# allenai/gpv-1

Hardware: AMD Instinct MI355X
Metric: images/sec/node (train step, 480x640, bs32/GPU) (higher is better)
Workload: dtype bf16; 1 GPU; GPV-1 (ResNet-50 + 6+6 DETR layers, 100 queries, RoI head, BERT-base, 3 co-attention, 3 text-decoder layers, V=10000) CocoCaptioning-only train step, dropout 0.1, AdamW; global_batch=32, image=480x640, parallelism=dp1

## Files before the change

gpv-1_amd/csrc/attention.hip:

```cpp
#include "common.h"
#include "../../include/gpv_hip.h"

namespace {

int g_bwd1_mode = tune_env("GPV_ATTN_BWD1", 1);
long g_bwd1_launches = 0;

struct AttnK {
  const void* q; const void* k; const void* v; void* o;
  int64_t q_bs, q_rs, k_bs, k_rs, v_bs, v_rs, o_bs, o_rs;
  int B, H, Sq, Sk, dh, skp, nsplit, sqp;
  float scale;
  const uint8_t* kpm; int causal;
  uint32_t dthresh; float dscale; uint64_t seed; const uint64_t* seed_dev;
  float* lse;
  const void* dout; int64_t do_bs, do_rs;
  void* dq; void* dk; void* dv;
};

constexpr uint32_t ATTN_PAIR_STEP = 0x9E3779B9u;
__device__ __forceinline__ uint32_t attn_row_seed(uint64_t seed, uint64_t row) { return hash_u32(seed, row); }
__device__ __forceinline__ uint32_t attn_pair_bits(uint32_t x) {
  x ^= x >> 16; x = __umul24(x, 0x85EBCBu);
  x ^= x >> 13; x = __umul24(x, 0xC2B2AFu);
  x ^= x >> 16;
  return x;
}
__device__ __forceinline__ int attn_ts(uint32_t dthresh) { return (int)(dthresh >> 16) - 32768; }
__device__ __forceinline__ bool attn_keep_lo(uint32_t w, int ts) { return (int)(short)(w & 0xffffu) >= ts; }
__device__ __forceinline__ bool attn_keep_hi(uint32_t w, int ts) { return ((int)w >> 16) >= ts; }
__device__ __forceinline__ uint32_t attn_drop_bits(uint32_t w, uint32_t ts2) {
  typedef short s16x2 __attribute__((ext_vector_type(2)));
// ... 1006 lines not shown
    T* dvp = reinterpret_cast<T*>(p.dv) + b * p.v_bs + (int64_t)key * p.v_rs + h * p.dh;
#pragma unroll
    for (int dt = 0; dt < DT; ++dt) {
      const int d = dt * 16 + g * 4;
      if (d < p.dh) {
        bf16x4 k4, v4;
#pragma unroll
        for (int i = 0; i < 4; ++i) { k4[i] = (bf16)dkacc[dt][i]; v4[i] = (bf16)dvacc[dt][i]; }
        *reinterpret_cast<bf16x4*>(dkp + d) = k4;
        *reinterpret_cast<bf16x4*>(dvp + d) = v4;
      }
    }
  }
}

template <int DHK, int DHV, int NQT, int NKT, bool CAUSAL>
__global__ __launch_bounds__(QTHR) void attn_bwd1_kernel(AttnK p) {
  using T = bf16;
  if (p.dthresh) p.seed = eff_seed(p.seed, p.seed_dev);
  constexpr int KP = DHK + 8, KC = DHK / 32, DT = DHV / 16, KTW = (NKT + QW - 1) / QW;
  const int sqp = p.sqp, QTP = sqp + 8, skp = p.skp, vtp = skp + 8;
  extern __shared__ __attribute__((aligned(16))) unsigned char smem_raw[];
  bf16* Qh = reinterpret_cast<bf16*>(smem_raw);
  bf16* Dh = Qh + sqp * KP;
  bf16* QTh = Dh + sqp * KP;
  bf16* DTh = QTh + DHV * QTP;
  bf16* KTh = DTh + DHV * QTP;
  bf16* dSb = KTh + DHV * vtp;
  float* lse_s = reinterpret_cast<float*>(dSb + 64 * vtp);
  float* del_s = lse_s + sqp;
  uint32_t* rs_s = reinterpret_cast<uint32_t*>(del_s + sqp);

// ... 14 lines not shown
    const int kt_ = wave + j * QW, key_ = kt_ * 16 + (lane & 15);
    const bool ok = kt_ < nkt && key_ < p.Sk;
#pragma unroll
    for (int kc = 0; kc < KC; ++kc) {
      const int d0 = kc * 32 + g * 8;
      AttnRaw8<T> a, c;
      if (ok && d0 < p.dh) { a.load(kg + (int64_t)key_ * p.k_rs + d0); c.load(vg + (int64_t)key_ * p.v_rs + d0); } else { a.zero(); c.zero(); }
      kh[j][kc] = a.r; vh[j][kc] = c.r;
    }
    kdead[j] = !ok || (p.kpm && p.kpm[(int64_t)b * p.Sk + key_] != 0);
  }

  const T* qg = reinterpret_cast<const T*>(p.q) + b * p.q_bs + h * p.dh;
  const T* dog = reinterpret_cast<const T*>(p.dout) + b * p.do_bs + h * p.dh;
  const T* og = reinterpret_cast<const T*>(p.o) + b * p.o_bs + h * p.dh;
  {
    RowBatch<T, DHK, NQT * 16, QTHR> qr, dr;
    ColBatch<T, DHV, NQT * 16, QTHR> qc, dc;
    qr.load(qg, p.q_rs, p.Sq, sqp, p.dh);
    dr.load(dog, p.do_rs, p.Sq, sqp, p.dh);
    qc.load(qg, p.q_rs, p.Sq, sqp);
    dc.load(dog, p.do_rs, p.Sq, sqp);
    qr.template store<false>(sqp, Qh, nullptr);
    dr.template store<false>(sqp, Dh, nullptr);
    qc.template store<false>(sqp, QTP, QTh, nullptr);
    dc.template store<false>(sqp, QTP, DTh, nullptr);
  }
  {
    ColBatch<T, DHV, NKT * 16, QTHR> kc_;
    kc_.load(kg, p.k_rs, p.Sk, skp);
    kc_.template store<false>(skp, vtp, KTh, nullptr);
  }
  for (int idx = threadIdx.x; idx < 8 * vtp; idx += QTHR)
    reinterpret_cast<bf16x8*>(dSb)[idx] = bf16x8{0, 0, 0, 0, 0, 0, 0, 0};
  for (int r = threadIdx.x; r < sqp; r += QTHR) {
    float dl = 0.f, ls = INFINITY;
    if (r < p.Sq) {
      const T* a = dog + (int64_t)r * p.do_rs;
      const T* c = og + (int64_t)r * p.o_rs;
      for (int d = 0; d < p.dh; d += 8) {
        float u[8], w[8];
        Ld8<T>::ld(a + d, u); Ld8<T>::ld(c + d, w);
#pragma unroll
        for (int e = 0; e < 8; ++e) dl += u[e] * w[e];
      }
      ls = p.lse[((int64_t)b * p.H + h) * p.Sq + r];
    }
    lse_s[r] = -ls * 1.4426950408889634f; del_s[r] = dl;
    rs_s[r] = p.dthresh ? attn_row_seed(p.seed, ((uint64_t)b * p.H + h) * p.Sq + r) : 0u;
  }
  __syncthreads();

  const float c2k = p.scale * 1.4426950408889634f;
// ... 195 lines not shown
  if (nsplit > (nkt + QW - 1) / QW) nsplit = (nkt + QW - 1) / QW;
  if (nsplit < 1) nsplit = 1;
  p.nsplit = nsplit;
  hipLaunchKernelGGL(fn, dim3(nsplit * bh), dim3(QTHR), lds, st, p);
  GPV_CHECK_LAUNCH();
  return 0;
}
template <int DHK, int DHV>
int launch_kv2(AttnK p, hipStream_t st) {
  if (p.Sq > 320) return -1;
  p.sqp = ((p.Sq + 31) / 32) * 32;
  if (p.sqp <= 128) return p.causal ? launch_kv2_c<DHK, DHV, 8, true>(p, st) : launch_kv2_c<DHK, DHV, 8, false>(p, st);
  return p.causal ? launch_kv2_c<DHK, DHV, 20, true>(p, st) : launch_kv2_c<DHK, DHV, 20, false>(p, st);
}

template <int DHK, int DHV, int NQT, int NKT, bool CAUSAL>
int launch_bwd1_c(AttnK p, hipStream_t st) {
  constexpr int KP = DHK + 8;
  const int QTP = p.sqp + 8, vtp = p.skp + 8;
  const size_t lds = ((size_t)2 * p.sqp * KP + (size_t)2 * DHV * QTP + (size_t)DHV * vtp + (size_t)64 * vtp) * 2 + (size_t)3 * p.sqp * sizeof(float);
  if (lds > 160 * 1024) return -1;
  auto fn = attn_bwd1_kernel<DHK, DHV, NQT, NKT, CAUSAL>;
  static size_t attr = 0;
  if (lds > 64 * 1024 && lds > attr) {
    hipError_t e = hipFuncSetAttribute(reinterpret_cast<const void*>(fn), hipFuncAttributeMaxDynamicSharedMemorySize, (int)lds);
    if (e != hipSuccess) { (void)hipGetLastError(); return (int)e; }
    attr = lds;
  }
  p.nsplit = 1;
  hipLaunchKernelGGL(fn, dim3(p.B * p.H), dim3(QTHR), lds, st, p);
  GPV_CHECK_LAUNCH();
  ++g_bwd1_launches;
  return 0;
}
template <int DHK, int DHV>
int launch_bwd1(AttnK p, hipStream_t st) {
  if (p.Sq > 320 || p.skp > 320) return -1;
  p.sqp = ((p.Sq + 31) / 32) * 32;
  const bool q8 = p.sqp <= 128, k8 = p.skp <= 128;
  if (p.causal) return (q8 && k8) ? launch_bwd1_c<DHK, DHV, 8, 8, true>(p, st) : -1;
  if (q8 && k8) return launch_bwd1_c<DHK, DHV, 8, 8, false>(p, st);
  if constexpr (DHK == 32) {
    if (q8) return launch_bwd1_c<DHK, DHV, 8, 20, false>(p, st);
    if (!k8) return launch_bwd1_c<DHK, DHV, 20, 20, false>(p, st);
  }
  return -1;
}
int dispatch_bwd1(const AttnK& p, hipStream_t st) {
  if (g_bwd1_mode == 0 || (g_bwd1_mode == 1 && p.B * p.H < 128)) return -1;
  switch (p.dh) {
    case 32: return launch_bwd1<32, 32>(p, st);
    case 48: return launch_bwd1<64, 48>(p, st);
    case 64: return launch_bwd1<64, 64>(p, st);
    case 96: return launch_bwd1<96, 96>(p, st);
// ... 609 lines not shown
  return elems * 2 * (sizeof(T) == 4 ? 2 : 1) + (size_t)p.skp * sizeof(float) <= 160 * 1024;
}

int fill(const gpv_attn_args* a, AttnK& p) {
  if (!a || !a->q || !a->k || !a->v || a->Sk <= 0 || a->Sq <= 0) return (int)hipErrorInvalidValue;
  p.q = a->q; p.k = a->k; p.v = a->v; p.o = a->o;
  p.q_bs = a->q_bs; p.q_rs = a->q_rs; p.k_bs = a->k_bs; p.k_rs = a->k_rs; p.v_bs = a->v_bs; p.v_rs = a->v_rs;
  p.o_bs = a->o_bs; p.o_rs = a->o_rs;
  p.B = a->B; p.H = a->H; p.Sq = a->Sq; p.Sk = a->Sk; p.dh = a->dh;
  p.skp = ((a->Sk + 63) / 64) * 64;
  p.scale = a->scale; p.kpm = a->kpm; p.causal = a->causal;
  p.dthresh = a->drop_p > 0.f ? drop_thresh(a->drop_p) : 0u;
  p.dscale = a->drop_p > 0.f ? 1.f / (1.f - a->drop_p) : 1.f;
  p.seed = a->seed; p.seed_dev = gpvk::g_seed_dev; p.lse = a->lse;
  p.dout = a->dout; p.do_bs = a->do_bs; p.do_rs = a->do_rs; p.dq = a->dq; p.dk = a->dk; p.dv = a->dv;
  return 0;
}
}

namespace gpvk {
int attn_bwd1_mode(int set) { const int prev = g_bwd1_mode; g_bwd1_mode = set; return prev; }
long attn_bwd1_launches(long set) { const long prev = g_bwd1_launches; if (set >= 0) g_bwd1_launches = set; return prev; }
}

extern "C" int gpv_attention_fwd(const gpv_attn_args* a, void* stream) {
  AttnK p{};
  int e = fill(a, p);
  if (e) return e;
  if (!a->o) return (int)hipErrorInvalidValue;
  hipStream_t st = reinterpret_cast<hipStream_t>(stream);
// ... 29 lines not shown
  if ((reinterpret_cast<uintptr_t>(a->q) | reinterpret_cast<uintptr_t>(a->k) | reinterpret_cast<uintptr_t>(a->o)) & 7) return (int)hipErrorInvalidValue;
  if (!a->v || (reinterpret_cast<uintptr_t>(a->v) & 1) || (reinterpret_cast<uintptr_t>(bias) & 3) || a->v_rs < a->H * a->dh || a->q_rs < a->H * a->dh ||
      a->k_rs < a->H * a->dh) return (int)hipErrorInvalidValue;
  QkvK xk{reinterpret_cast<const bf16*>(xp), reinterpret_cast<const bf16*>(x), x_bs, x_rs, reinterpret_cast<const bf16*>(w), bias};
  hipStream_t st = reinterpret_cast<hipStream_t>(stream);
  if (p.skp <= 128) return p.skp == 128 ? launch_qkv<8, true>(p, xk, st) : launch_qkv<8, false>(p, xk, st);
  return p.skp == 320 ? launch_qkv<20, true>(p, xk, st) : launch_qkv<20, false>(p, xk, st);
}

extern "C" int gpv_attention_bwd(const gpv_attn_args* a, void* stream) {
  AttnK p{};
  int e = fill(a, p);
  if (e) return e;
  if (!a->o || !a->dout || !a->dq || !a->dk || !a->dv || !a->lse) return (int)hipErrorInvalidValue;
  hipStream_t st = reinterpret_cast<hipStream_t>(stream);
  const bool f32 = a->dtype == GPV_F32;
  if (!(f32 ? q_short_fits<float, 1>(p) : q_short_fits<bf16, 1>(p))) {
    e = f32 ? dispatch_long<float, 1>(p, st) : dispatch_long<bf16, 1>(p, st);
    if (e) return e;
    return f32 ? dispatch_kvl<float>(p, st) : dispatch_kvl<bf16>(p, st);
  }
  if (a->dtype != GPV_F32) {
    e = dispatch_bwd1(p, st);
    if (e >= 0) return e;
  }
  e = a->dtype == GPV_F32 ? dispatch_q<float, 1>(p, st) : dispatch_q<bf16, 1>(p, st);
  if (e) return e;
  return a->dtype == GPV_F32 ? dispatch_kv<float>(p, st) : dispatch_kv<bf16>(p, st);
}
```

gpv-1_amd/hip.py:

```python
import ctypes as C
import os
import threading

import torch

BF16, F32 = 0, 1
ACT_NONE, ACT_RELU, ACT_GELU = 0, 1, 2
KMAJOR, TRANS = 0, 1

_LIB = None
TUNING = os.environ.get('GPV_TUNING_LIB', '0') == '1'
_LIB_PATH = os.environ.get('GPV_HIP_LIB') or os.path.join(os.path.dirname(os.path.abspath(__file__)), 'csrc',
                                                          'libgpv_hip_tuning.so' if TUNING else 'libgpv_hip.so')


class GemmArgs(C.Structure):
    _fields_ = [('A', C.c_void_p), ('B', C.c_void_p), ('C', C.c_void_p),
                ('M', C.c_int), ('N', C.c_int), ('K', C.c_int), ('batch', C.c_int),
                ('lda', C.c_int64), ('ldb', C.c_int64), ('ldc', C.c_int64),
                ('sA', C.c_int64), ('sB', C.c_int64), ('sC', C.c_int64),
                ('layoutA', C.c_int), ('layoutB', C.c_int), ('dtype_in', C.c_int), ('dtype_out', C.c_int),
                ('alpha', C.c_float), ('rowscale', C.c_void_p), ('bias', C.c_void_p),
                ('res', C.c_void_p), ('ldr', C.c_int64), ('sR', C.c_int64),
                ('relu_mask', C.c_void_p), ('ldm', C.c_int64),
# ... 9 lines not shown
                ('KH', C.c_int), ('KW', C.c_int), ('SH', C.c_int), ('SW', C.c_int), ('PH', C.c_int), ('PW', C.c_int),
                ('dtype_in', C.c_int), ('dtype_out', C.c_int),
                ('rowscale', C.c_void_p), ('bias', C.c_void_p), ('res', C.c_void_p), ('relu_mask', C.c_void_p),
                ('act', C.c_int), ('split_k', C.c_int), ('workspace', C.c_void_p), ('workspace_bytes', C.c_int64),
                ('y_mask_bits', C.c_void_p), ('relu_mask_bits', C.c_void_p)]


class AttnArgs(C.Structure):
    _fields_ = [('q', C.c_void_p), ('k', C.c_void_p), ('v', C.c_void_p), ('o', C.c_void_p),
                ('q_bs', C.c_int64), ('q_rs', C.c_int64), ('k_bs', C.c_int64), ('k_rs', C.c_int64),
                ('v_bs', C.c_int64), ('v_rs', C.c_int64), ('o_bs', C.c_int64), ('o_rs', C.c_int64),
                ('B', C.c_int), ('H', C.c_int), ('Sq', C.c_int), ('Sk', C.c_int), ('dh', C.c_int),
                ('scale', C.c_float), ('kpm', C.c_void_p), ('causal', C.c_int),
                ('drop_p', C.c_float), ('seed', C.c_uint64), ('lse', C.c_void_p), ('dtype', C.c_int),
                ('dout', C.c_void_p), ('do_bs', C.c_int64), ('do_rs', C.c_int64),
                ('dq', C.c_void_p), ('dk', C.c_void_p), ('dv', C.c_void_p)]


class TTProblem(C.Structure):
    _fields_ = [('A', C.c_void_p), ('B', C.c_void_p), ('C', C.c_void_p), ('a_rowsum', C.c_void_p),
                ('M', C.c_int), ('N', C.c_int), ('K', C.c_int), ('lda', C.c_int), ('ldb', C.c_int), ('ldc', C.c_int)]


class FoldProblem(C.Structure):
    _fields_ = [('partials', C.c_void_p), ('out0', C.c_void_p), ('out1', C.c_void_p), ('nblk', C.c_int), ('cols', C.c_int)]


class ConvWgradProblem(C.Structure):
    _fields_ = [('x', C.c_void_p), ('dy', C.c_void_p), ('dw', C.c_void_p), ('rowscale', C.c_void_p)] + \
               [(k, C.c_int) for k in ('B', 'IH', 'IW', 'Cs', 'Cin', 'OH', 'OW', 'Cout', 'KH', 'KW', 'SH', 'SW', 'PH', 'PW')]

# ... 305 lines not shown
        raise ValueError('attention_qkv_fwd: xp and x must share one row layout (the library takes ONE pair of strides for both)')
    a = _attn_args(q, k, v, o, strides, B, H, S, S, 32, scale, kpm, False, drop_p, seed, lse)
    _chk(lib().gpv_attention_qkv_fwd(C.byref(a), _p(xp), _p(x), C.c_int64(S * x.stride(0)), C.c_int64(x.stride(0)), _p(w), _p(_f32(bias)),
                                     _stream()), 'gpv_attention_qkv_fwd')


def attention_bwd(q, k, v, o, dout, dq, dk, dv, strides, do_strides, B, H, Sq, Sk, dh, scale, kpm=None,
                  causal=False, drop_p=0.0, seed=0, lse=None):
    a = _attn_args(q, k, v, o, strides, B, H, Sq, Sk, dh, scale, kpm, causal, drop_p, seed, lse)
    a.dout = _p(dout)
    a.do_bs, a.do_rs = do_strides
    a.dq, a.dk, a.dv = _p(dq), _p(dk), _p(dv)
    _chk(lib().gpv_attention_bwd(C.byref(a), _stream()), 'gpv_attention_bwd')


def linear_layernorm_fwd(a, w, bias, x, gamma, beta, s, y, mean, rstd, rows, eps, drop_p=0.0, seed=0, pos=None, y2=None):
    if (pos is None) != (y2 is None):
        raise ValueError('pos and y2 come together')
    if any(t.dtype != torch.bfloat16 for t in (a, w, x, s, y)):
        raise TypeError('linear_layernorm_fwd: bf16 activations and weight')
    _chk(lib().gpv_linear_layernorm_fwd(_p(a), _p(w), _p(_f32(bias)), _p(x), _p(_f32(gamma)), _p(_f32(beta)), _p(s), _p(y), _p(_f32(mean)),
                                        _p(_f32(rstd)), C.c_int(rows), C.c_int(w.shape[1]), C.c_int(w.shape[0]), C.c_float(eps), C.c_float(drop_p), C.c_uint64(seed),
                                        _p(pos), C.c_int(0 if pos is None else pos.numel() // w.shape[0]), _p(y2), _stream()), 'gpv_linear_layernorm_fwd')


def layernorm_fwd(x, s, gamma, beta, y, mean, rstd, rows, cols, eps, drop_p=0.0, seed=0, pos=None, y2=None):
    if (pos is None) != (y2 is None):
        raise ValueError('layernorm_fwd: pos and y2 come together')
    if pos is not None and (pos.dtype != x.dtype or y2.dtype != x.dtype or pos.numel() % cols != 0):
        raise TypeError('layernorm_fwd: pos / y2 in the activation dtype, whole rows')
# ... 314 lines not shown
```

gpv-1_amd/ops.py:

```python
import math

import os
import weakref

import torch
from torch.autograd import Function

from . import hip

ACT_NONE, ACT_RELU, ACT_GELU = hip.ACT_NONE, hip.ACT_RELU, hip.ACT_GELU


class Runtime:
    def __init__(self):
        self.dtype = torch.bfloat16
        self.weights_epoch = 0
        self.static_epoch = 0
        self.seed = 0x5EED
        self.seed_explicit = False
        self._ctr = 0
        self.cache = {}
        self.backward_milestone = None
        self.split = None
        self.seed_dev = None
# ... 786 lines not shown
            elif dsr is not None and ds is None:
                dxr = dxr.clone()
            dxr = ch.done(dxr)
        return ((dxr if ctx.needs_input_grad[0] else None), (dsr if ctx.needs_input_grad[1] else None)) + (None,) * (nin - 2)


PROJ_LN = os.environ.get('GPV_PROJ_LN', '1') != '0'
PROJ_LN_MIN_ROWS = int(os.environ.get('GPV_PROJ_LN_MIN_ROWS', '2048'))


def proj_layernorm_ok(w, x):
    return (PROJ_LN and RT.dtype == torch.bfloat16 and w.K == 256 and w.N == 256 and x.shape[-1] == 256 and w.bias is not None
            and x.numel() // 256 >= PROJ_LN_MIN_ROWS)


class ProjAddLayerNormFn(Function):

    @staticmethod
    def forward(ctx, x, a, w, gamma, beta, eps, drop_p, chain=None, pos=None, pos_param=None):
        ctx.chain = chain.join() if (chain is not None and ctx.needs_input_grad[0]) else None
        ctx.set_materialize_grads(False)
        cols = x.shape[-1]
        x2 = _c(_as_compute(x)).reshape(-1, cols)
        a2 = _c(_as_compute(a)).reshape(-1, w.K)
        rows = x2.shape[0]
        s2 = torch.empty_like(x2)
        y = torch.empty_like(x2)
        mean = torch.empty(rows, device=x.device, dtype=torch.float32)
        rstd = torch.empty_like(mean)
        seed = RT.next_seed() if drop_p > 0 else 0
# ... 11 lines not shown
    @staticmethod
    def backward(ctx, dy, dy2=None):
        nin = 10
        if dy is None and dy2 is None:
            return (None,) * nin
        x2, s2, mean, rstd, a2 = ctx.saved_tensors
        rows, cols = x2.shape
        if dy2 is not None:
            _pos_sink(ctx.pos_param, _c(_as_compute(dy2)).reshape(rows, cols), rows, cols)
        d1, d2 = _two_grads(dy, dy2, rows, cols)
        dx = torch.empty_like(x2)
        ds = torch.empty_like(x2) if ctx.drop_p > 0 else None
        _ln_backward(d1, d2, x2, s2, ctx.gamma, ctx.beta, mean, rstd, dx, ds, rows, cols, ctx.drop_p, ctx.seed)
        dxr = dx.reshape(ctx.shape)
        if ctx.chain is not None and ctx.needs_input_grad[0]:
            ch = ctx.chain
            if ch.acc is not None:
                t = torch.empty_like(dx)
                hip.add(dx, _c(ch.acc).reshape(rows, cols), t, t.numel())
                dxr = t.reshape(ctx.shape)
            elif ds is None:
                dxr = dxr.clone()
            dxr = ch.done(dxr)
        da = _linear_backward(ctx.w, a2, ds if ds is not None else dx, None, ctx.needs_input_grad[1], ctx.ashape)
        return ((dxr if ctx.needs_input_grad[0] else None), da) + (None,) * (nin - 2)


def proj_add_layernorm(x, a, w, gamma, beta, eps, drop_p=0.0, chain=None, pos=None, pos_param=None):
    return ProjAddLayerNormFn.apply(x, a, w, gamma, beta, eps, drop_p, chain, pos, pos_param)


FFN_FUSED = os.environ.get('GPV_FFN_FUSED', '0') == '1'


class FFNBlockFn(Function):

    @staticmethod
    def forward(ctx, x, w1, w2, gamma, beta, eps, drop_p, pos=None, pos_param=None):
# ... 157 lines not shown

    @staticmethod
    def backward(ctx, do):
        w, B, H, S, kpm, drop_p = ctx.meta[:6]
        E = w.K
        xp2, x2, qk, v, o, lse = ctx.saved_tensors
        do = _c(_as_compute(do))
        dqk, dv = torch.empty_like(qk), torch.empty_like(v)
        hip.attention_bwd(qk[:, :E], qk[:, E:], v, o, do, dqk[:, :E], dqk[:, E:], dv, ctx.st, (S * E, E), B, H, S, S, E // H, ctx.scale,
                          kpm=kpm, drop_p=drop_p, seed=ctx.seed, lse=lse)
        dx = _linear_backward(W(w.weight, w.bias, 2 * E, 3 * E), x2, dv, ctx.cv, ctx.needs_input_grad[2], ctx.x_shape)
        dxp = _linear_backward(W(w.weight, w.bias, 0, 2 * E), xp2, dqk, ctx.cq, ctx.needs_input_grad[1], ctx.xp_shape)
        return None, dxp, dx, None


def attention_qkv(xp, x, w, B, H, S, kpm=None, drop_p=0.0, chains=(None, None)):
    dummy = None
    if torch.is_grad_enabled() and not (xp.requires_grad or x.requires_grad) and (w.weight.requires_grad or (w.bias is not None and w.bias.requires_grad)):
        dummy = _dummy(x.device)
    return SelfAttnQKVFn.apply((w, B, H, S, kpm, drop_p, chains[0], chains[1]), xp, x, dummy)


class AddFn(Function):

    @staticmethod
    def forward(ctx, a, b):
        ctx.set_materialize_grads(False)
        a2, b2 = _c(_as_compute(a)), _c(_as_compute(b))
        y = torch.empty_like(a2)
        cols = a2.shape[-1]
# ... 169 lines not shown
```

gpv-1_amd/transformer.py:

```python
import os

import torch
import torch.nn as nn

from . import ops
from .ops import W

HOIST_KV = os.environ.get('GPV_HOIST_KV', '1') != '0'


class LinearP(nn.Module):

    def __init__(self, in_features, out_features, bias=True):
        super().__init__()
        ref = nn.Linear(in_features, out_features, bias=bias)
        self.weight = nn.Parameter(ref.weight.detach().clone())
        self.bias = nn.Parameter(ref.bias.detach().clone()) if bias else None
        self.in_features, self.out_features = in_features, out_features

    def forward(self, x, act=ops.ACT_NONE, drop_p=0.0, out_f32=False, chain=None):
        return ops.linear(x, W(self.weight, self.bias), act, drop_p, out_f32, chain)


def ffn_block(x, l1, l2, norm, drop_p, pos=None, pos_param=None):
# ... 19 lines not shown

class MultiheadAttention(nn.Module):

    def __init__(self, embed_dim, num_heads, dropout=0.0):
        super().__init__()
        self.embed_dim, self.num_heads, self.dropout = embed_dim, num_heads, dropout
        self.head_dim = embed_dim // num_heads
        self.in_proj_weight = nn.Parameter(torch.empty(3 * embed_dim, embed_dim))
        self.in_proj_bias = nn.Parameter(torch.zeros(3 * embed_dim))
        self.out_proj = LinearP(embed_dim, embed_dim)
        nn.init.xavier_uniform_(self.in_proj_weight)
        nn.init.constant_(self.out_proj.bias, 0.)

    def forward(self, q_in, k_in, v_in, B, Sq, Sk, key_padding_mask=None, causal=False, chains=(None, None, None), kv=None, out_drop=0.0,
                no_proj=False):
        E = self.embed_dim
        w, b = self.in_proj_weight, self.in_proj_bias
        cq, ck, cv = chains
        if kv is not None:
            k_all, kcol, v_all, vcol, sk, sv = kv
            q = ops.linear(q_in, W(w, b, 0, E), chain=cq)
            if k_all is v_all:
                bufs, roles, sinks = [q, k_all], ((0, 0), (1, kcol), (1, vcol)), (None, sk)
            else:
                bufs, roles, sinks = [q, k_all, v_all], ((0, 0), (1, kcol), (2, vcol)), (None, sk, sv)
            o = ops.attention(bufs, roles, B, self.num_heads, Sq, Sk, self.head_dim, kpm=key_padding_mask,
                              causal=causal, drop_p=self.dropout if self.training else 0.0,
                              sinks=sinks if (sk is not None or sv is not None) else None)
            return o if no_proj else self.out_proj(o, drop_p=out_drop)
        if q_in is k_in and k_in is v_in:
            bufs = [ops.linear(q_in, W(w, b, 0, 3 * E), chain=cq)]
            roles = ((0, 0), (0, E), (0, 2 * E))
        elif q_in is k_in:
            if Sq == Sk and ops.attention_qkv_ok(E, self.num_heads, Sq, causal, B):
                o = ops.attention_qkv(q_in, v_in, W(w, b, 0, 3 * E), B, self.num_heads, Sq, kpm=key_padding_mask,
                                      drop_p=self.dropout if self.training else 0.0, chains=(cq, cv))
                return o if no_proj else self.out_proj(o, drop_p=out_drop)
            bufs = [ops.linear(q_in, W(w, b, 0, 2 * E), chain=cq), ops.linear(v_in, W(w, b, 2 * E, 3 * E), chain=cv)]
            roles = ((0, 0), (0, E), (1, 0))
        elif k_in is v_in:
            bufs = [ops.linear(q_in, W(w, b, 0, E), chain=cq), ops.linear(k_in, W(w, b, E, 3 * E), chain=ck)]
            roles = ((0, 0), (1, 0), (1, E))
        else:
            bufs = [ops.linear(q_in, W(w, b, 0, E), chain=cq), ops.linear(k_in, W(w, b, E, 2 * E), chain=ck),
                    ops.linear(v_in, W(w, b, 2 * E, 3 * E), chain=cv)]
            roles = ((0, 0), (1, 0), (2, 0))
        o = ops.attention(bufs, roles, B, self.num_heads, Sq, Sk, self.head_dim, kpm=key_padding_mask, causal=causal,
                          drop_p=self.dropout if self.training else 0.0)
        return o if no_proj else self.out_proj(o, drop_p=out_drop)


class TransformerEncoderLayer(nn.Module):
    def __init__(self, d_model, nhead, dim_feedforward=2048, dropout=0.1):
        super().__init__()
        self.self_attn = MultiheadAttention(d_model, nhead, dropout=dropout)
        self.linear1 = LinearP(d_model, dim_feedforward)
        self.linear2 = LinearP(dim_feedforward, d_model)
        self.norm1 = LayerNormP(d_model)
        self.norm2 = LayerNormP(d_model)
        self.p = dropout

    def forward(self, src, qk, pos, B, S, kpm):
        p = self.p if self.training else 0.0
        ch = ops.grad_chain(src)
        o = self.self_attn(qk, qk, src, B, S, S, kpm, chains=(ch, ch, ch), no_proj=True)
        src = self.norm1.proj(src, o, self.self_attn.out_proj, p, chain=ch)
        return ffn_block(src, self.linear1, self.linear2, self.norm2, p, pos=pos)

    def forward_pre(self, src, pos, B, S, kpm, pos_grad=False):
        p = self.p if self.training else 0.0
        if pos_grad:
            s2 = self.norm1(src)
            qk = ops.add(s2, pos)
        else:
            s2, qk = self.norm1(src, pos=pos)
        src = ops.add(src, self.self_attn(qk, qk, s2, B, S, S, kpm, out_drop=p))
        s2 = self.norm2(src)
        return ops.add(src, self.linear2(self.linear1(s2, ops.ACT_RELU, p), drop_p=p))


class TransformerDecoderLayer(nn.Module):
    def __init__(self, d_model, nhead, dim_feedforward=2048, dropout=0.1):
        super().__init__()
        self.self_attn = MultiheadAttention(d_model, nhead, dropout=dropout)
        self.multihead_attn = MultiheadAttention(d_model, nhead, dropout=dropout)
        self.linear1 = LinearP(d_model, dim_feedforward)
        self.linear2 = LinearP(dim_feedforward, d_model)
        self.norm1 = LayerNormP(d_model)
        self.norm2 = LayerNormP(d_model)
        self.norm3 = LayerNormP(d_model)
        self.p = dropout

    def forward(self, tgt, tgt_qp, memory, mem_pos, qpos, qpos_param, B, Q, S, kpm, mem_chain=None, emit=True, kv=None):
        p = self.p if self.training else 0.0
        ch = ops.grad_chain(tgt)
        o = self.self_attn(tgt_qp, tgt_qp, tgt, B, Q, Q, chains=(None, None, ch), no_proj=True)
        tgt, tq = self.norm1.proj(tgt, o, self.self_attn.out_proj, p, chain=ch, pos=qpos, pos_param=qpos_param)
        a = self.multihead_attn(tq, mem_pos, memory, B, Q, S, kpm, chains=(None, mem_chain, mem_chain), kv=kv, no_proj=True)
        tgt = self.norm2.proj(tgt, a, self.multihead_attn.out_proj, p)
        if not emit:
            return ffn_block(tgt, self.linear1, self.linear2, self.norm3, p), None
        return ffn_block(tgt, self.linear1, self.linear2, self.norm3, p, pos=qpos, pos_param=qpos_param)

    def forward_pre(self, tgt, memory, mem_pos, qpos, qpos_param, B, Q, S, kpm):
        p = self.p if self.training else 0.0
        t2, tq = self.norm1(tgt, pos=qpos, pos_param=qpos_param)
        tgt = ops.add(tgt, self.self_attn(tq, tq, t2, B, Q, Q, out_drop=p))
        t2, tq = self.norm2(tgt, pos=qpos, pos_param=qpos_param)
        tgt = ops.add(tgt, self.multihead_attn(tq, mem_pos, memory, B, Q, S, kpm, out_drop=p))
        t2 = self.norm3(tgt)
        return ops.add(tgt, self.linear2(self.linear1(t2, ops.ACT_RELU, p), drop_p=p))


class TransformerEncoder(nn.Module):
# ... 124 lines not shown
```

include/gpv_hip.h:

```cpp
#ifndef GPV_HIP_H
#define GPV_HIP_H
#include <stdint.h>
#ifdef __cplusplus
extern "C" {
#endif

#define GPV_BF16 0
#define GPV_F32 1

#define GPV_ACT_NONE 0
#define GPV_ACT_RELU 1
#define GPV_ACT_GELU 2

#define GPV_KMAJOR 0
#define GPV_TRANS 1

int gpv_abi_version(void);
int gpv_build_id(char* buf, int cap);

#define GPV_TT_GROUP_MAX 48
typedef struct {
  const void* A; const void* B; float* C; float* a_rowsum;
  int M, N, K;
  int lda, ldb, ldc;
// ... 122 lines not shown
#endif
int gpv_stem_pool(const void* x, const void* w, const float* shift, void* y, int B, int Hp, int Wp, int CH, int CW, int PH, int PW,
                  void* stream);

typedef struct {
  const void* q; const void* k; const void* v; void* o;
  int64_t q_bs, q_rs, k_bs, k_rs, v_bs, v_rs, o_bs, o_rs;
  int B, H, Sq, Sk, dh;
  float scale;
  const uint8_t* kpm; int causal;
  float drop_p; uint64_t seed;
  float* lse;
  int dtype;
  const void* dout; int64_t do_bs, do_rs;
  void* dq; void* dk; void* dv;
} gpv_attn_args;
int gpv_attention_fwd(const gpv_attn_args* a, void* stream);
int gpv_attention_bwd(const gpv_attn_args* a, void* stream);
int gpv_attention_qkv_fwd(const gpv_attn_args* a, const void* xp, const void* x, int64_t x_bs, int64_t x_rs, const void* w,
                          const float* bias, void* stream);

int gpv_layernorm_fwd(const void* x, const void* s, const float* gamma, const float* beta, void* y,
                      float* mean, float* rstd, int rows, int cols, float eps, float drop_p,
                      uint64_t seed, int dtype, void* stream);
int gpv_layernorm_bwd(const void* dy, const void* x, const void* s, const float* gamma,
                      const float* mean, const float* rstd, void* dx, void* ds, float* dgamma,
                      float* dbeta, int rows, int cols, float drop_p, uint64_t seed, int dtype,
                      void* stream);
int gpv_layernorm_pos_fwd(const void* x, const void* s, const float* gamma, const float* beta, void* y, float* mean, float* rstd,
                          int rows, int cols, float eps, float drop_p, uint64_t seed, const void* pos, int pos_rows, void* y2,
                          int dtype, void* stream);
// ... 71 lines not shown
```

Baseline: 2142 images/sec.

## Fuse out-projection input-gradient GEMM into attention backward prologue

Adds a PROJ variant of the attention backward kernel that computes dO = dZ·Wo^T per head inside the prologue with MFMA, so the separate dx GEMM and the dO round trip through global memory go away. A new autograd function, AttnSublayerFn, wraps attention, the out-projection and the residual LayerNorm as one sublayer for the encoder and decoder layers. Each block now rereads the full 256-wide dZ row and a slice of the weight, which adds redundant loads across heads. The PROJ path only applies to bf16 attention with 8 heads of 32, non-causal, and sequence lengths up to 320; other cases fall back to the old path.

```diff
diff --git a/gpv-1_amd/csrc/attention.hip b/gpv-1_amd/csrc/attention.hip
--- a/gpv-1_amd/csrc/attention.hip
+++ b/gpv-1_amd/csrc/attention.hip
@@ -16,6 +16,7 @@
   float* lse;
   const void* dout; int64_t do_bs, do_rs;
   void* dq; void* dk; void* dv;
+  const void* wt;
 };
 
 constexpr uint32_t ATTN_PAIR_STEP = 0x9E3779B9u;
@@ -1052,8 +1053,9 @@
   }
 }
 
-template <int DHK, int DHV, int NQT, int NKT, bool CAUSAL>
+template <int DHK, int DHV, int NQT, int NKT, bool CAUSAL, bool PROJ = false>
 __global__ __launch_bounds__(QTHR) void attn_bwd1_kernel(AttnK p) {
+  static_assert(!PROJ || (DHK == 32 && DHV == 32 && !CAUSAL), "the projection prologue is built for 8 heads of 32");
   using T = bf16;
   if (p.dthresh) p.seed = eff_seed(p.seed, p.seed_dev);
   constexpr int KP = DHK + 8, KC = DHK / 32, DT = DHV / 16, KTW = (NKT + QW - 1) / QW;
@@ -1098,7 +1100,54 @@
   const T* qg = reinterpret_cast<const T*>(p.q) + b * p.q_bs + h * p.dh;
   const T* dog = reinterpret_cast<const T*>(p.dout) + b * p.do_bs + h * p.dh;
   const T* og = reinterpret_cast<const T*>(p.o) + b * p.o_bs + h * p.dh;
-  {
+  if constexpr (PROJ) {
+    constexpr int KD = 256, KCX = KD / 32, NR = (NQT + QW - 1) / QW;
+    const int li = lane & 15, nqt = sqp >> 4;
+    RowBatch<T, DHK, NQT * 16, QTHR> qr;
+    ColBatch<T, DHV, NQT * 16, QTHR> qc;
+    qr.load(qg, p.q_rs, p.Sq, sqp, p.dh);
+    qc.load(qg, p.q_rs, p.Sq, sqp);
+    const T* wg = reinterpret_cast<const T*>(p.wt) + (int64_t)(h * 32 + li) * KD + g * 8;
+    const T* zg = reinterpret_cast<const T*>(p.dout) + b * p.do_bs + g * 8;
+    bf16x8 wf[2][KCX], nz[KCX];
+#pragma unroll
+    for (int dt = 0; dt < 2; ++dt)
+#pragma unroll
+      for (int kc = 0; kc < KCX; ++kc) wf[dt][kc] = *reinterpret_cast<const bf16x8*>(wg + dt * 16 * KD + kc * 32);
+    auto fetch = [&](int t) {
+      const T* zr = zg + (int64_t)min(t * 16 + li, p.Sq - 1) * p.do_rs;
+#pragma unroll
+      for (int kc = 0; kc < KCX; ++kc) nz[kc] = *reinterpret_cast<const bf16x8*>(zr + kc * 32);
+    };
+    fetch(wave);
+    qr.template store<false>(sqp, Qh, nullptr);
+    qc.template store<false>(sqp, QTP, QTh, nullptr);
+#pragma unroll
+    for (int r = 0; r < NR; ++r) {
+      const int t = wave + r * QW;
+      if (t < nqt) {
+        bf16x8 zf[KCX];
+#pragma unroll
+        for (int kc = 0; kc < KCX; ++kc) zf[kc] = nz[kc];
+        if (r + 1 < NR) fetch(t + QW);
+        f32x4 acc[2] = {f32x4{0.f, 0.f, 0.f, 0.f}, f32x4{0.f, 0.f, 0.f, 0.f}};
+#pragma unroll
+        for (int kc = 0; kc < KCX; ++kc)
+#pragma unroll
+          for (int dt = 0; dt < 2; ++dt) acc[dt] = mfma16(wf[dt][kc], zf[kc], acc[dt]);
+        const int q = t * 16 + li;
+#pragma unroll
+        for (int dt = 0; dt < 2; ++dt) {
+          bf16x4 d4;
+#pragma unroll
+          for (int i = 0; i < 4; ++i) d4[i] = q < p.Sq ? (bf16)acc[dt][i] : (bf16)0.f;
+          *reinterpret_cast<bf16x4*>(Dh + q * KP + dt * 16 + g * 4) = d4;
+#pragma unroll
+          for (int i = 0; i < 4; ++i) DTh[(dt * 16 + g * 4 + i) * QTP + q] = d4[i];
+        }
+      }
+    }
+  } else {
     RowBatch<T, DHK, NQT * 16, QTHR> qr, dr;
     ColBatch<T, DHV, NQT * 16, QTHR> qc, dc;
     qr.load(qg, p.q_rs, p.Sq, sqp, p.dh);
@@ -1117,10 +1166,11 @@
   }
   for (int idx = threadIdx.x; idx < 8 * vtp; idx += QTHR)
     reinterpret_cast<bf16x8*>(dSb)[idx] = bf16x8{0, 0, 0, 0, 0, 0, 0, 0};
+  if constexpr (PROJ) __syncthreads();
   for (int r = threadIdx.x; r < sqp; r += QTHR) {
     float dl = 0.f, ls = INFINITY;
     if (r < p.Sq) {
-      const T* a = dog + (int64_t)r * p.do_rs;
+      const T* a = PROJ ? Dh + r * KP : dog + (int64_t)r * p.do_rs;
       const T* c = og + (int64_t)r * p.o_rs;
       for (int d = 0; d < p.dh; d += 8) {
         float u[8], w[8];
@@ -1346,13 +1396,13 @@
   return p.causal ? launch_kv2_c<DHK, DHV, 20, true>(p, st) : launch_kv2_c<DHK, DHV, 20, false>(p, st);
 }
 
-template <int DHK, int DHV, int NQT, int NKT, bool CAUSAL>
+template <int DHK, int DHV, int NQT, int NKT, bool CAUSAL, bool PROJ = false>
 int launch_bwd1_c(AttnK p, hipStream_t st) {
   constexpr int KP = DHK + 8;
   const int QTP = p.sqp + 8, vtp = p.skp + 8;
   const size_t lds = ((size_t)2 * p.sqp * KP + (size_t)2 * DHV * QTP + (size_t)DHV * vtp + (size_t)64 * vtp) * 2 + (size_t)3 * p.sqp * sizeof(float);
   if (lds > 160 * 1024) return -1;
-  auto fn = attn_bwd1_kernel<DHK, DHV, NQT, NKT, CAUSAL>;
+  auto fn = attn_bwd1_kernel<DHK, DHV, NQT, NKT, CAUSAL, PROJ>;
   static size_t attr = 0;
   if (lds > 64 * 1024 && lds > attr) {
     hipError_t e = hipFuncSetAttribute(reinterpret_cast<const void*>(fn), hipFuncAttributeMaxDynamicSharedMemorySize, (int)lds);
@@ -1370,6 +1420,15 @@
   if (p.Sq > 320 || p.skp > 320) return -1;
   p.sqp = ((p.Sq + 31) / 32) * 32;
   const bool q8 = p.sqp <= 128, k8 = p.skp <= 128;
+  if (p.wt) {
+    if constexpr (DHK == 32) {
+      if (p.causal) return -1;
+      if (q8 && k8) return launch_bwd1_c<DHK, DHV, 8, 8, false, true>(p, st);
+      if (q8) return launch_bwd1_c<DHK, DHV, 8, 20, false, true>(p, st);
+      if (!k8) return launch_bwd1_c<DHK, DHV, 20, 20, false, true>(p, st);
+    }
+    return -1;
+  }
   if (p.causal) return (q8 && k8) ? launch_bwd1_c<DHK, DHV, 8, 8, true>(p, st) : -1;
   if (q8 && k8) return launch_bwd1_c<DHK, DHV, 8, 8, false>(p, st);
   if constexpr (DHK == 32) {
@@ -2009,6 +2068,7 @@
   p.dscale = a->drop_p > 0.f ? 1.f / (1.f - a->drop_p) : 1.f;
   p.seed = a->seed; p.seed_dev = gpvk::g_seed_dev; p.lse = a->lse;
   p.dout = a->dout; p.do_bs = a->do_bs; p.do_rs = a->do_rs; p.dq = a->dq; p.dk = a->dk; p.dv = a->dv;
+  p.wt = nullptr;
   return 0;
 }
 }
@@ -2068,6 +2128,15 @@
   if (e) return e;
   if (!a->o || !a->dout || !a->dq || !a->dk || !a->dv || !a->lse) return (int)hipErrorInvalidValue;
   hipStream_t st = reinterpret_cast<hipStream_t>(stream);
+  if (a->proj_wt) {
+    if (a->dtype != GPV_BF16 || a->dh != 32 || a->H * a->dh != 256 || a->Sq > 320 || a->Sk > 320 || a->causal || a->proj_ld != 256)
+      return GPV_NOT_TAKEN;
+    if ((a->do_rs & 7) || (a->do_bs & 7) || a->do_rs < 256 || a->do_bs < (int64_t)a->Sq * a->do_rs) return (int)hipErrorInvalidValue;
+    if ((reinterpret_cast<uintptr_t>(a->dout) | reinterpret_cast<uintptr_t>(a->proj_wt)) & 15) return (int)hipErrorInvalidValue;
+    p.wt = a->proj_wt;
+    e = dispatch_bwd1(p, st);
+    return e >= 0 ? e : GPV_NOT_TAKEN;
+  }
   const bool f32 = a->dtype == GPV_F32;
   if (!(f32 ? q_short_fits<float, 1>(p) : q_short_fits<bf16, 1>(p))) {
     e = f32 ? dispatch_long<float, 1>(p, st) : dispatch_long<bf16, 1>(p, st);
diff --git a/gpv-1_amd/hip.py b/gpv-1_amd/hip.py
--- a/gpv-1_amd/hip.py
+++ b/gpv-1_amd/hip.py
@@ -47,7 +47,8 @@
                 ('scale', C.c_float), ('kpm', C.c_void_p), ('causal', C.c_int),
                 ('drop_p', C.c_float), ('seed', C.c_uint64), ('lse', C.c_void_p), ('dtype', C.c_int),
                 ('dout', C.c_void_p), ('do_bs', C.c_int64), ('do_rs', C.c_int64),
-                ('dq', C.c_void_p), ('dk', C.c_void_p), ('dv', C.c_void_p)]
+                ('dq', C.c_void_p), ('dk', C.c_void_p), ('dv', C.c_void_p),
+                ('proj_wt', C.c_void_p), ('proj_ld', C.c_int64)]
 
 
 class TTProblem(C.Structure):
@@ -383,6 +384,27 @@
     _chk(lib().gpv_attention_bwd(C.byref(a), _stream()), 'gpv_attention_bwd')
 
 
+NOT_TAKEN = -1
+
+
+def attention_bwd_proj(q, k, v, o, dz, wt, dq, dk, dv, strides, B, H, Sq, Sk, dh, scale, kpm=None, causal=False, drop_p=0.0, seed=0,
+                       lse=None):
+    if dz.dim() != 2 or wt.dim() != 2 or dz.stride(1) != 1 or wt.stride(1) != 1 or dz.dtype != q.dtype or wt.dtype != q.dtype:
+        return False
+    if dz.shape[0] != B * Sq or dz.shape[1] != H * dh or tuple(wt.shape) != (H * dh, H * dh):
+        return False
+    a = _attn_args(q, k, v, o, strides, B, H, Sq, Sk, dh, scale, kpm, causal, drop_p, seed, lse)
+    a.dout = _p(dz)
+    a.do_bs, a.do_rs = Sq * dz.stride(0), dz.stride(0)
+    a.dq, a.dk, a.dv = _p(dq), _p(dk), _p(dv)
+    a.proj_wt, a.proj_ld = _p(wt), wt.stride(0)
+    err = lib().gpv_attention_bwd(C.byref(a), _stream())
+    if err == NOT_TAKEN:
+        return False
+    _chk(err, 'gpv_attention_bwd (proj)')
+    return True
+
+
 def linear_layernorm_fwd(a, w, bias, x, gamma, beta, s, y, mean, rstd, rows, eps, drop_p=0.0, seed=0, pos=None, y2=None):
     if (pos is None) != (y2 is None):
         raise ValueError('pos and y2 come together')
diff --git a/gpv-1_amd/ops.py b/gpv-1_amd/ops.py
--- a/gpv-1_amd/ops.py
+++ b/gpv-1_amd/ops.py
@@ -824,6 +824,17 @@
             and x.numel() // 256 >= PROJ_LN_MIN_ROWS)
 
 
+def _residual_grad(ch, dx, dx_is_dz, shape):
+    dxr = dx.reshape(shape)
+    if ch.acc is not None:
+        t = torch.empty_like(dx)
+        hip.add(dx, _c(ch.acc).reshape(dx.shape), t, t.numel())
+        dxr = t.reshape(shape)
+    elif dx_is_dz:
+        dxr = dxr.clone()
+    return ch.done(dxr)
+
+
 class ProjAddLayerNormFn(Function):
 
     @staticmethod
@@ -865,14 +876,7 @@
         _ln_backward(d1, d2, x2, s2, ctx.gamma, ctx.beta, mean, rstd, dx, ds, rows, cols, ctx.drop_p, ctx.seed)
         dxr = dx.reshape(ctx.shape)
         if ctx.chain is not None and ctx.needs_input_grad[0]:
-            ch = ctx.chain
-            if ch.acc is not None:
-                t = torch.empty_like(dx)
-                hip.add(dx, _c(ch.acc).reshape(rows, cols), t, t.numel())
-                dxr = t.reshape(ctx.shape)
-            elif ds is None:
-                dxr = dxr.clone()
-            dxr = ch.done(dxr)
+            dxr = _residual_grad(ctx.chain, dx, ds is None, ctx.shape)
         da = _linear_backward(ctx.w, a2, ds if ds is not None else dx, None, ctx.needs_input_grad[1], ctx.ashape)
         return ((dxr if ctx.needs_input_grad[0] else None), da) + (None,) * (nin - 2)
 
@@ -1060,6 +1064,120 @@
         return None, dxp, dx, None
 
 
+ATTN_PROJ_BWD = os.environ.get('GPV_ATTN_PROJ_BWD', '1') != '0'
+
+
+def attention_proj_ok(E, H, Sq, Sk, causal, B):
+    return (ATTN_PROJ_BWD and RT.dtype == torch.bfloat16 and E == 256 and H == 8 and 0 < Sq <= 320 and 0 < Sk <= 320 and not causal
+            and B * H >= 64)
+
+
+class AttnSublayerFn(Function):
+
+    @staticmethod
+    def forward(ctx, meta, x, dummy, *ins):
+        front, w, gamma, beta, eps, drop_p, chain, pos, pos_param = meta
+        E = w.K
+        if front[0] == 'qkv':
+            _, wi, B, H, Sq, kpm, adrop, chain_qk, chain_v = front
+            Sk, dh = Sq, E // H
+            xp2 = _c(_as_compute(ins[0])).reshape(-1, E)
+            xv2 = _c(_as_compute(ins[1])).reshape(-1, E)
+            M = xp2.shape[0]
+            qk = torch.empty(M, 2 * E, device=xp2.device, dtype=RT.dtype)
+            v = torch.empty(M, E, device=xp2.device, dtype=RT.dtype)
+            bufs, roles = (qk, v), ((0, 0), (0, E), (1, 0))
+            ctx.cq = chain_qk.join() if (chain_qk is not None and ctx.needs_input_grad[3]) else None
+            ctx.cv = chain_v.join() if (chain_v is not None and ctx.needs_input_grad[4]) else None
+            ctx.in_shapes = (ins[0].shape, ins[1].shape)
+            extra = (xp2, xv2)
+        else:
+            _, roles, B, H, Sq, Sk, dh, kpm, adrop, sinks = front
+            bufs = tuple(_c(_as_compute(b)) for b in ins)
+            extra = ()
+        (qi, qo), (ki, ko), (vi, vo) = roles
+        qb, kb, vb = bufs[qi], bufs[ki], bufs[vi]
+        o = torch.empty(B * Sq, E, device=qb.device, dtype=RT.dtype)
+        lse = torch.empty(B, H, Sq, device=qb.device, dtype=torch.float32)
+        st = ((Sq * qb.shape[1], qb.shape[1]), (Sk * kb.shape[1], kb.shape[1]), (Sk * vb.shape[1], vb.shape[1]), (Sq * E, E))
+        aseed = RT.next_seed() if adrop > 0 else 0
+        scale = 1.0 / math.sqrt(dh)
+        if front[0] == 'qkv':
+            hip.attention_qkv_fwd(xp2, xv2, wi.lp(), wi.bias_f32(), qk[:, :E], qk[:, E:], v, o, st, B, H, Sq, scale, kpm=kpm, drop_p=adrop,
+                                  seed=aseed, lse=lse)
+        else:
+            hip.attention_fwd(qb[:, qo:], kb[:, ko:], vb[:, vo:], o, st, B, H, Sq, Sk, dh, scale, kpm=kpm, drop_p=adrop, seed=aseed, lse=lse)
+        ctx.chain = chain.join() if (chain is not None and ctx.needs_input_grad[1]) else None
+        ctx.set_materialize_grads(False)
+        x2 = _c(_as_compute(x)).reshape(-1, E)
+        rows = x2.shape[0]
+        s2 = torch.empty_like(x2)
+        y = torch.empty_like(x2)
+        mean = torch.empty(rows, device=x.device, dtype=torch.float32)
+        rstd = torch.empty_like(mean)
+        seed = RT.next_seed() if drop_p > 0 else 0
+        p2 = None if pos is None else _pos_rows(pos, E)
+        y2 = None if pos is None else torch.empty_like(x2)
+        hip.linear_layernorm_fwd(o, w.lp(), w.bias_f32(), x2, None if gamma is None else gamma.detach(), None if beta is None else beta.detach(),
+                                 s2, y, mean, rstd, rows, eps, drop_p, seed, pos=p2, y2=y2)
+        ctx.meta, ctx.aseed, ctx.seed, ctx.st, ctx.scale, ctx.shape, ctx.nbuf = meta, aseed, seed, st, scale, x.shape, len(bufs)
+        ctx.geom = (roles, B, H, Sq, Sk, dh, kpm, adrop)
+        ctx.save_for_backward(x2, s2, mean, rstd, o, lse, *bufs, *extra)
+        if pos is None:
+            return y.reshape(x.shape)
+        return y.reshape(x.shape), y2.reshape(x.shape)
+
+    @staticmethod
+    def backward(ctx, dy, dy2=None):
+        front, w, gamma, beta, eps, drop_p, _, _, pos_param = ctx.meta
+        nin = 3 + (2 if front[0] == 'qkv' else ctx.nbuf)
+        if dy is None and dy2 is None:
+            return (None,) * nin
+        x2, s2, mean, rstd, o, lse, *rest = ctx.saved_tensors
+        bufs, extra = rest[:ctx.nbuf], rest[ctx.nbuf:]
+        roles, B, H, Sq, Sk, dh, kpm, adrop = ctx.geom
+        rows, cols = x2.shape
+        if dy2 is not None:
+            _pos_sink(pos_param, _c(_as_compute(dy2)).reshape(rows, cols), rows, cols)
+        d1, d2 = _two_grads(dy, dy2, rows, cols)
+        dx = torch.empty_like(x2)
+        ds = torch.empty_like(x2) if drop_p > 0 else None
+        _ln_backward(d1, d2, x2, s2, gamma, beta, mean, rstd, dx, ds, rows, cols, drop_p, ctx.seed)
+        dxr = dx.reshape(ctx.shape)
+        if ctx.chain is not None and ctx.needs_input_grad[1]:
+            dxr = _residual_grad(ctx.chain, dx, ds is None, ctx.shape)
+        dz = ds if ds is not None else dx
+        _linear_backward(w, o, dz, None, False, None)
+        (qi, qo), (ki, ko), (vi, vo) = roles
+        sinks = front[9] if (front[0] == 'bufs' and front[9] is not None) else (None,) * len(bufs)
+        grads = [torch.empty_like(b) if s is None else s.slot(b) for b, s in zip(bufs, sinks)]
+        q, k, v = bufs[qi][:, qo:], bufs[ki][:, ko:], bufs[vi][:, vo:]
+        dq, dk, dv = grads[qi][:, qo:], grads[ki][:, ko:], grads[vi][:, vo:]
+        akw = dict(kpm=kpm, drop_p=adrop, seed=ctx.aseed, lse=lse)
+        if not (w.mirror_ok() and hip.attention_bwd_proj(q, k, v, o, dz, w.lpT(), dq, dk, dv, ctx.st, B, H, Sq, Sk, dh, ctx.scale, **akw)):
+            do = torch.empty_like(o)
+            w.dx_gemm(dz, do, rows)
+            hip.attention_bwd(q, k, v, o, do, dq, dk, dv, ctx.st, (Sq * cols, cols), B, H, Sq, Sk, dh, ctx.scale, **akw)
+        gx = dxr if ctx.needs_input_grad[1] else None
+        if front[0] == 'qkv':
+            wi, E = front[1], cols
+            xp2, xv2 = extra
+            dxv = _linear_backward(W(wi.weight, wi.bias, 2 * E, 3 * E), xv2, grads[1], ctx.cv, ctx.needs_input_grad[4], ctx.in_shapes[1])
+            dxp = _linear_backward(W(wi.weight, wi.bias, 0, 2 * E), xp2, grads[0], ctx.cq, ctx.needs_input_grad[3], ctx.in_shapes[0])
+            return None, gx, None, dxp, dxv
+        for s_ in sinks:
+            if s_ is not None:
+                s_.note_writer()
+        return (None, gx, None, *[g if s is None else s.wrote() for g, s in zip(grads, sinks)])
+
+
+def attn_sublayer(front, x, ins, w, gamma, beta, eps, drop_p=0.0, chain=None, pos=None, pos_param=None):
+    dummy = None
+    if torch.is_grad_enabled() and not (x.requires_grad or any(t.requires_grad for t in ins)):
+        dummy = _dummy(x.device)
+    return AttnSublayerFn.apply((front, w, gamma, beta, eps, drop_p, chain, pos, pos_param), x, dummy, *ins)
+
+
 def attention_qkv(xp, x, w, B, H, S, kpm=None, drop_p=0.0, chains=(None, None)):
     dummy = None
     if torch.is_grad_enabled() and not (xp.requires_grad or x.requires_grad) and (w.weight.requires_grad or (w.bias is not None and w.bias.requires_grad)):
diff --git a/gpv-1_amd/transformer.py b/gpv-1_amd/transformer.py
--- a/gpv-1_amd/transformer.py
+++ b/gpv-1_amd/transformer.py
@@ -57,6 +57,18 @@
 
     def forward(self, q_in, k_in, v_in, B, Sq, Sk, key_padding_mask=None, causal=False, chains=(None, None, None), kv=None, out_drop=0.0,
                 no_proj=False):
+        adrop = self.dropout if self.training else 0.0
+        bufs, roles, sinks = self._project(q_in, k_in, v_in, B, Sq, Sk, causal, chains, kv)
+        if bufs is None:
+            E = self.embed_dim
+            o = ops.attention_qkv(q_in, v_in, W(self.in_proj_weight, self.in_proj_bias, 0, 3 * E), B, self.num_heads, Sq,
+                                  kpm=key_padding_mask, drop_p=adrop, chains=(chains[0], chains[2]))
+        else:
+            o = ops.attention(bufs, roles, B, self.num_heads, Sq, Sk, self.head_dim, kpm=key_padding_mask, causal=causal, drop_p=adrop,
+                              sinks=sinks)
+        return o if no_proj else self.out_proj(o, drop_p=out_drop)
+
+    def _project(self, q_in, k_in, v_in, B, Sq, Sk, causal, chains, kv):
         E = self.embed_dim
         w, b = self.in_proj_weight, self.in_proj_bias
         cq, ck, cv = chains
@@ -67,30 +79,34 @@
                 bufs, roles, sinks = [q, k_all], ((0, 0), (1, kcol), (1, vcol)), (None, sk)
             else:
                 bufs, roles, sinks = [q, k_all, v_all], ((0, 0), (1, kcol), (2, vcol)), (None, sk, sv)
-            o = ops.attention(bufs, roles, B, self.num_heads, Sq, Sk, self.head_dim, kpm=key_padding_mask,
-                              causal=causal, drop_p=self.dropout if self.training else 0.0,
-                              sinks=sinks if (sk is not None or sv is not None) else None)
-            return o if no_proj else self.out_proj(o, drop_p=out_drop)
+            return bufs, roles, sinks if (sk is not None or sv is not None) else None
         if q_in is k_in and k_in is v_in:
-            bufs = [ops.linear(q_in, W(w, b, 0, 3 * E), chain=cq)]
-            roles = ((0, 0), (0, E), (0, 2 * E))
-        elif q_in is k_in:
+            return [ops.linear(q_in, W(w, b, 0, 3 * E), chain=cq)], ((0, 0), (0, E), (0, 2 * E)), None
+        if q_in is k_in:
             if Sq == Sk and ops.attention_qkv_ok(E, self.num_heads, Sq, causal, B):
-                o = ops.attention_qkv(q_in, v_in, W(w, b, 0, 3 * E), B, self.num_heads, Sq, kpm=key_padding_mask,
-                                      drop_p=self.dropout if self.training else 0.0, chains=(cq, cv))
-                return o if no_proj else self.out_proj(o, drop_p=out_drop)
-            bufs = [ops.linear(q_in, W(w, b, 0, 2 * E), chain=cq), ops.linear(v_in, W(w, b, 2 * E, 3 * E), chain=cv)]
-            roles = ((0, 0), (0, E), (1, 0))
-        elif k_in is v_in:
-            bufs = [ops.linear(q_in, W(w, b, 0, E), chain=cq), ops.linear(k_in, W(w, b, E, 3 * E), chain=ck)]
-            roles = ((0, 0), (1, 0), (1, E))
-        else:
-            bufs = [ops.linear(q_in, W(w, b, 0, E), chain=cq), ops.linear(k_in, W(w, b, E, 2 * E), chain=ck),
-                    ops.linear(v_in, W(w, b, 2 * E, 3 * E), chain=cv)]
-            roles = ((0, 0), (1, 0), (2, 0))
-        o = ops.attention(bufs, roles, B, self.num_heads, Sq, Sk, self.head_dim, kpm=key_padding_mask, causal=causal,
-                          drop_p=self.dropout if self.training else 0.0)
-        return o if no_proj else self.out_proj(o, drop_p=out_drop)
+                return None, None, None
+            return [ops.linear(q_in, W(w, b, 0, 2 * E), chain=cq), ops.linear(v_in, W(w, b, 2 * E, 3 * E), chain=cv)], ((0, 0), (0, E), (1, 0)), None
+        if k_in is v_in:
+            return [ops.linear(q_in, W(w, b, 0, E), chain=cq), ops.linear(k_in, W(w, b, E, 3 * E), chain=ck)], ((0, 0), (1, 0), (1, E)), None
+        return ([ops.linear(q_in, W(w, b, 0, E), chain=cq), ops.linear(k_in, W(w, b, E, 2 * E), chain=ck),
+                 ops.linear(v_in, W(w, b, 2 * E, 3 * E), chain=cv)], ((0, 0), (1, 0), (2, 0)), None)
+
+    def sublayer(self, norm, x, q_in, k_in, v_in, B, Sq, Sk, key_padding_mask=None, chains=(None, None, None), kv=None, drop_p=0.0,
+                 chain=None, pos=None, pos_param=None):
+        E, H = self.embed_dim, self.num_heads
+        wo = W(self.out_proj.weight, self.out_proj.bias)
+        if not (torch.is_grad_enabled() and ops.attention_proj_ok(E, H, Sq, Sk, False, B) and ops.proj_layernorm_ok(wo, x)
+                and (pos is None or ops.LN_POS)):
+            o = self.forward(q_in, k_in, v_in, B, Sq, Sk, key_padding_mask, chains=chains, kv=kv, no_proj=True)
+            return norm.proj(x, o, self.out_proj, drop_p, chain=chain, pos=pos, pos_param=pos_param)
+        adrop = self.dropout if self.training else 0.0
+        bufs, roles, sinks = self._project(q_in, k_in, v_in, B, Sq, Sk, False, chains, kv)
+        if bufs is None:
+            front = ('qkv', W(self.in_proj_weight, self.in_proj_bias, 0, 3 * E), B, H, Sq, key_padding_mask, adrop, chains[0], chains[2])
+            bufs = (q_in, v_in)
+        else:
+            front = ('bufs', roles, B, H, Sq, Sk, self.head_dim, key_padding_mask, adrop, sinks)
+        return ops.attn_sublayer(front, x, bufs, wo, norm.weight, norm.bias, norm.eps, drop_p, chain, pos, pos_param)
 
 
 class TransformerEncoderLayer(nn.Module):
@@ -106,8 +122,7 @@
     def forward(self, src, qk, pos, B, S, kpm):
         p = self.p if self.training else 0.0
         ch = ops.grad_chain(src)
-        o = self.self_attn(qk, qk, src, B, S, S, kpm, chains=(ch, ch, ch), no_proj=True)
-        src = self.norm1.proj(src, o, self.self_attn.out_proj, p, chain=ch)
+        src = self.self_attn.sublayer(self.norm1, src, qk, qk, src, B, S, S, kpm, chains=(ch, ch, ch), drop_p=p, chain=ch)
         return ffn_block(src, self.linear1, self.linear2, self.norm2, p, pos=pos)
 
     def forward_pre(self, src, pos, B, S, kpm, pos_grad=False):
@@ -137,10 +152,10 @@
     def forward(self, tgt, tgt_qp, memory, mem_pos, qpos, qpos_param, B, Q, S, kpm, mem_chain=None, emit=True, kv=None):
         p = self.p if self.training else 0.0
         ch = ops.grad_chain(tgt)
-        o = self.self_attn(tgt_qp, tgt_qp, tgt, B, Q, Q, chains=(None, None, ch), no_proj=True)
-        tgt, tq = self.norm1.proj(tgt, o, self.self_attn.out_proj, p, chain=ch, pos=qpos, pos_param=qpos_param)
-        a = self.multihead_attn(tq, mem_pos, memory, B, Q, S, kpm, chains=(None, mem_chain, mem_chain), kv=kv, no_proj=True)
-        tgt = self.norm2.proj(tgt, a, self.multihead_attn.out_proj, p)
+        tgt, tq = self.self_attn.sublayer(self.norm1, tgt, tgt_qp, tgt_qp, tgt, B, Q, Q, chains=(None, None, ch), drop_p=p, chain=ch,
+                                          pos=qpos, pos_param=qpos_param)
+        tgt = self.multihead_attn.sublayer(self.norm2, tgt, tq, mem_pos, memory, B, Q, S, kpm, chains=(None, mem_chain, mem_chain),
+                                           kv=kv, drop_p=p)
         if not emit:
             return ffn_block(tgt, self.linear1, self.linear2, self.norm3, p), None
         return ffn_block(tgt, self.linear1, self.linear2, self.norm3, p, pos=qpos, pos_param=qpos_param)
diff --git a/include/gpv_hip.h b/include/gpv_hip.h
--- a/include/gpv_hip.h
+++ b/include/gpv_hip.h
@@ -160,7 +160,9 @@
   int dtype;
   const void* dout; int64_t do_bs, do_rs;
   void* dq; void* dk; void* dv;
+  const void* proj_wt; int64_t proj_ld;
 } gpv_attn_args;
+#define GPV_NOT_TAKEN (-1)
 int gpv_attention_fwd(const gpv_attn_args* a, void* stream);
 int gpv_attention_bwd(const gpv_attn_args* a, void* stream);
 int gpv_attention_qkv_fwd(const gpv_attn_args* a, const void* xp, const void* x, int64_t x_bs, int64_t x_rs, const void* w,
```

New measurement: 2129 images/sec. About the same (-0.6%).
